# swift-nav/albatross

Hardware: AMD Instinct MI355X
Metric: GP fits/sec (Gram+Chol+solve) at N=16384 fp64 (higher is better)
Workload: dtype f64

## Files before the change

albatross_amd/csrc/chol.hip:

```cpp
#include <cstdlib>
#include "common.h"
#include "mfma_f64.h"
#include "gemm_tiles.h"
#include "trsm_kernel.h"
#include "pub.h"

namespace agp {
void launch_set_identity_batched(hipStream_t s, double *B, long long ld, long long stride, long long m, long long count);

__device__ __forceinline__ double readlane_f64(double v, int lane) {
  const long long b = __double_as_longlong(v);
  const int lo = __builtin_amdgcn_readlane((int)(b & 0xffffffffll), lane);
  const int hi = __builtin_amdgcn_readlane((int)(b >> 32), lane);
  return __longlong_as_double(((long long)hi << 32) | (unsigned int)lo);
}

__device__ __forceinline__ double rsqrt_nr(double x) {
  double y = __builtin_amdgcn_rsq(x);
  const double h = 0.5 * x;
  y = y * (1.5 - h * y * y);
  y = y * (1.5 - h * y * y);
  return y;
}

// ... 699 lines not shown
  p.A = A; p.lda = lda; p.k0 = k0; p.nbk = nbk;
  p.img = img + (k0 / NB) * (long long)IMG_DOUBLES;
  p.y = y ? y + k0 : nullptr;
  p.flags = flags; p.scalars = scalars;
  hipLaunchKernelGGL(potrf_diag_kernel, dim3(1), dim3(256), 0, s, p);
}

static void timed_gemm(hipStream_t s, FactorTimers *timers, double *C, long long lda, const double *P,
                       const double *Q, long long M, long long N, long long K, bool bulk, int variant = -1,
                       const float *P32 = nullptr, long long ld32 = 0) {
  if (!bulk) {
    launch_gemm_nt_sub(s, C, lda, P, lda, false, Q, lda, false, M, N, K, true);
    return;
  }
  BulkTiming bt;
  const bool timed = timers && timers->ev && timers->used + 2 <= timers->n_ev;
  if (timed) { bt.e0 = timers->ev[timers->used]; bt.e1 = timers->ev[timers->used + 1]; }
  if (variant >= 0) launch_trailing_update_as(variant, s, C, lda, P, Q, lda, M, K, timed ? &bt : nullptr, P32, P32, ld32);
  else launch_trailing_update(s, C, lda, P, Q, lda, M, K, timed ? &bt : nullptr);
  if (timed && bt.flops > 0.) {
    timers->flops[timers->used / 2] = bt.flops;
    timers->used += 2;
  }
}

constexpr long long FUSED_BELOW = 4608;
constexpr long long INNER_LEFT_ABOVE = 6144;
constexpr long long NBO_512_ABOVE = 2048, NBO_256_ABOVE = 1024;
constexpr long long NBO_WIDE_ABOVE = 8192;
constexpr long long THROTTLE_BELOW = 8192;
constexpr long long U1_F32_ABOVE = 4096;
constexpr long long SINGLE_BELOW = 1536;
constexpr long long MASK_BELOW = 8704;

static long long step_slots(agp_context *ctx) {
  if (ctx->step_slots <= 0) {
    int per_cu = 0;
    if (hipOccupancyMaxActiveBlocksPerMultiprocessor(&per_cu, panel_fused_kernel<true>, 256, 0) != hipSuccess || per_cu <= 0) {
      (void)hipGetLastError();
      per_cu = 1;
    }
    ctx->step_slots = (long long)per_cu * ctx->cus;
  }
  return ctx->step_slots;
}

static bool step_fits(agp_context *ctx, long long rows) {
  return ctx->tune.step_below > 0 && rows <= ctx->tune.step_below && step_slots(ctx) >= 10 + rows / 64 + 64;
}

__global__ __launch_bounds__(256) void prep_kernel(PrepArgs a) {
  int e = 0;
  while (e + 1 < a.n && (long long)blockIdx.x >= a.first_block[e + 1]) ++e;
  const long long i0 = ((long long)blockIdx.x - a.first_block[e]) * 1024 + threadIdx.x;
  unsigned long long *d = a.dst[e];
  const unsigned long long *sr = a.src[e];
  const unsigned long long pat = a.pattern[e];
#pragma unroll
  for (int u = 0; u < 4; ++u) {
    const long long i = i0 + 256 * u;
    if (i < a.count[e]) d[i] = sr ? sr[i] : pat;
  }
}

__global__ __launch_bounds__(256) void copy_table_kernel(const CopyItem *__restrict__ table) {
  const CopyItem it = table[blockIdx.y];
// ... 35 lines not shown
    ctx->d_dpub = nullptr;
    ctx->d_rowcnt = nullptr;
    ctx->dpub_cap = 0;
    const long long cap = (b1 + 31) / 32 * 32;
    if (hipMalloc(&ctx->d_dpub, sizeof(double) * (size_t)cap * (IMG_DOUBLES + 2)) == hipSuccess) {
      ctx->dpub_cap = cap;
      ctx->d_rowcnt = reinterpret_cast<unsigned long long *>(ctx->d_dpub + cap * (long long)IMG_DOUBLES);
    }
    else (void)hipGetLastError();
  }
  const long long cnt_img = (b1 - b0) * (long long)IMG_DOUBLES, cnt_z = k_end - k_begin;
  if (ctx->d_dpub && ctx->dpub_cap >= b1) {
    prep->fill(ctx->d_rowcnt + 2 * b0, 0ull, 2 * (b1 - b0));
    prep->sentinel(ctx->d_dpub + b0 * (long long)IMG_DOUBLES, cnt_img);
  }
  prep->sentinel(invd + b0 * (long long)IMG_DOUBLES, cnt_img);
  prep->sentinel(ctx->d_zpub + k_begin, cnt_z);
  if (want_step && k_begin == 0 && ctx->d_headcnt && ctx->tune.merge_above > 0 && k_end > ctx->tune.merge_above && !prep->full()) {
    prep->fill(ctx->d_headcnt, 0ull, agp_context::HEADCNT_WORDS);
    ctx->headcnt_ready = true;
  }
  ctx->zpub_ready_n = k_end;
  ctx->img_ready = invd;
  return true;
}

void panel_fused_prepare(agp_context *ctx, hipStream_t s, double *invd, long long k_begin, long long k_end, bool want_step) {
  PrepArgs prep;
  if (panel_fused_plan(ctx, invd, k_begin, k_end, want_step, &prep)) launch_prep(s, prep);
}

static void panel_phase(agp_context *ctx, hipStream_t s, double *A, long long n, long long lda, double *invd,
                        double *y, long long K0, long long kend, FactorTimers *timers, bool step_mode = false,
                        long long mark_after = -1, hipEvent_t mark_event = nullptr) {
  if (kend != n) step_mode = false;
  const bool inner_left = !step_mode && (n - K0) > INNER_LEFT_ABOVE;
  const bool fused = ctx->tune.panel_fused && ctx->d_zpub && ctx->zpub_ready_n >= kend && ctx->img_ready == invd &&
                     ((n - K0) <= FUSED_BELOW || step_mode);
  for (long long k = K0; k < kend; k += NB) {
    const int nbk = (int)((n - k < NB) ? n - k : NB);
    if (mark_event && k == mark_after + NB) (void)hipEventRecord(mark_event, s);
    if (inner_left && k > K0) {
      const double *P = A + K0 * lda + k;
      timed_gemm(s, timers, A + k * lda + k, lda, P, P, n - k, nbk, k - K0, false);
    }
    const long long below = n - (k + nbk);
    if (fused) {
      PotrfArgs pa;
      pa.A = A; pa.lda = lda; pa.k0 = k; pa.nbk = nbk;
      pa.img = invd + (k / NB) * (long long)IMG_DOUBLES;
      pa.y = y ? y + k : nullptr;
      pa.flags = ctx->d_flags; pa.scalars = ctx->d_scalars;
      pa.zpub = y ? ctx->d_zpub + k : nullptr;
      pa.below = below > 0 ? below : 0;
      if (step_mode && k > K0) {
        pa.dpub = ctx->d_dpub + (k / NB) * (long long)IMG_DOUBLES;
        unsigned grid = (unsigned)(1 + UPD_BLOCKS + (pa.below + 63) / 64);
        if (pa.below > 0) {
          const long long nt = (pa.below + 63) / 64;
          pa.trail_first = grid;
          pa.rowcnt = ctx->d_rowcnt + (k + NB) / 64;
          pa.rowcnt_expect = 2ull * (unsigned long long)((k - K0) / NB);
          const long long tiles = nt * (nt + 1) / 2 + 2 * nt;
          const long long slots = step_slots(ctx), first_round = ctx->cus, ncrit = grid;
          long long workers = tiles, nhold = 0;
          if (ncrit + workers > first_round && ncrit < first_round) {
            nhold = tiles <= 1200 ? ncrit : 1 + UPD_BLOCKS;
            const long long cap = slots - ncrit - nhold;
            if (workers > cap) workers = cap;
            if (ncrit + workers <= first_round) nhold = 0;
          } else if (workers > slots - ncrit) {
            workers = slots - ncrit;
          }
          if (workers < 2 * nt) workers = 2 * nt < tiles ? 2 * nt : tiles;
          pa.trail_tiles = tiles;
          pa.trail_workers = workers;
          grid += (unsigned)workers;
          if (nhold > 0) {
            pa.hold_index = (unsigned)first_round;
            pa.hold_count = (unsigned)nhold;
            grid += (unsigned)nhold;
          }
        }
        hipLaunchKernelGGL(panel_fused_kernel<true>, dim3(grid), dim3(256), 0, s, pa);
        ++ctx->sched.panels_step;
      } else {
        hipLaunchKernelGGL(panel_fused_kernel<false>, dim3((unsigned)(1 + (pa.below + 63) / 64)), dim3(256), 0, s, pa);
        ++ctx->sched.panels_fused;
      }
      if (below <= 0) continue;
    } else {
      launch_potrf(s, A, lda, k, nbk, invd, y, ctx->d_flags, ctx->d_scalars);
      ++ctx->sched.panels_split;
      if (below <= 0) continue;
      TrsmArgs t;
      t.img = invd + (k / NB) * (long long)IMG_DOUBLES;
      t.nbk = nbk;
      t.Y = A + k * lda + (k + nbk);
      t.stride_m = lda; t.stride_n = 1;
      t.ncols = below;
      t.z = y ? y + k : nullptr;
      t.yrest = y ? y + k + nbk : nullptr;
      t.batch_img = t.batch_Y = 0; t.n_total = 0;
      const unsigned grid = (unsigned)((below + 63) / 64);
      if (y) hipLaunchKernelGGL((trsm_micro_kernel<false, true>), dim3(grid), dim3(256), 0, s, t);
      else hipLaunchKernelGGL((trsm_micro_kernel<false, false>), dim3(grid), dim3(256), 0, s, t);
    }
    const long long width = kend - (k + nbk);
    if (width > 0 && !inner_left && !(step_mode && fused)) {
      const double *P = A + k * lda + (k + nbk);
      timed_gemm(s, timers, A + (k + nbk) * lda + (k + nbk), lda, P, P, below, width, nbk, false);
    }
  }
}

__global__ __launch_bounds__(64) void head_gate_kernel(const unsigned long long *done, unsigned long long expect, int *flags) {
  if (threadIdx.x == 0) {
    const unsigned long long t0 = __builtin_amdgcn_s_memrealtime();
    for (int spin = 1; __hip_atomic_load(done, __ATOMIC_RELAXED, __HIP_MEMORY_SCOPE_AGENT) < expect; ++spin) {
      if ((spin & 63) == 0 && poll_expired(t0, flags)) break;
      __builtin_amdgcn_s_sleep(16);
    }
    __atomic_thread_fence(__ATOMIC_ACQUIRE);
  }
}

void launch_head_gate(hipStream_t s, const unsigned long long *done, unsigned long long expect, int *flags) {
  hipLaunchKernelGGL(head_gate_kernel, dim3(1), dim3(64), 0, s, done, expect, flags);
}

static bool host_wait_event(hipEvent_t ev) {
  for (;;) {
    const hipError_t e = hipEventQuery(ev);
    if (e == hipSuccess) return true;
    if (e != hipErrorNotReady) { (void)hipGetLastError(); return false; }
    for (int i = 0; i < 32; ++i) __builtin_ia32_pause();
  }
}
// ... 127 lines not shown
      unsigned short *dst = reinterpret_cast<unsigned short *>(ctx->p32) + (size_t)(p32_flip ? 1 : 0) * (ctx->p32_bytes / sizeof(unsigned short) / 2);
      p32_flip = !p32_flip;
      launch_convert_panel_bf16x3(sa, P, lda, n - kend, K, dst);
      P16 = dst;
    } else if (variant == 5 && ctx->p32 && (n - kend) >= U1_F32_ABOVE && f16x2_depth_ok(K) && 2 * f16x2_bytes(n - kend, K) <= ctx->p32_bytes) {
      unsigned short *dst = reinterpret_cast<unsigned short *>(ctx->p32) + (size_t)(p32_flip ? 1 : 0) * (ctx->p32_bytes / sizeof(unsigned short) / 2);
      p32_flip = !p32_flip;
      launch_convert_panel_f16x2(sa, P, lda, n - kend, K, rs16 + kend, dst);
      P16 = dst;
    }
    (void)hipEventRecord(ctx->ev_a, sa);
    const bool merged = variant <= 0 && nbo_fixed == 0 && !step && next_end < n && ctx->headcnt_ready && ctx->tune.merge_above > 0 &&
                        (n - kend) > ctx->tune.merge_above && step_index < agp_context::HEADCNT_WORDS && (next_end - kend) % NB == 0;
    if (merged) {
      sb = (ctx->stream_masked && (n - kend) <= MASK_BELOW) ? ctx->stream_masked : ctx->stream2;
      if (sb != sb_prev && have_u2) (void)hipStreamWaitEvent(sb, ctx->ev_b, 0);
      sb_prev = sb;
      (void)hipStreamWaitEvent(sb, ctx->ev_a, 0);
      BulkTiming bt;
      const bool timed = timers && timers->ev && timers->used + 2 <= timers->n_ev;
      if (timed) { bt.e0 = timers->ev[timers->used]; bt.e1 = timers->ev[timers->used + 1]; }
      long long head_tiles = 0;
      unsigned long long *cnt = ctx->d_headcnt + step_index;
      launch_trailing_update_merged(sb, A + kend * lda + kend, lda, P, lda, n - kend, K, (int)((next_end - kend) / NB), cnt, &head_tiles,
                                    timed ? &bt : nullptr);
      if (timed && bt.flops > 0.) {
        timers->flops[timers->used / 2] = bt.flops;
        timers->used += 2;
      }
      (void)hipEventRecord(ctx->ev_b, sb);
      have_u2 = true;
      launch_head_gate(sa, cnt, (unsigned long long)head_tiles, ctx->d_flags);
      rec.add_step(next_end, rec.MERGED | (sb == ctx->stream_masked ? rec.MASKED : 0u));
      panel_phase(ctx, sa, A, n, lda, invd, y, kend, next_end, timers, false);
      K0 = kend;
      kend = next_end;
      ++step_index;
      continue;
    }
    ++step_index;
    if (have_u2) (void)hipStreamWaitEvent(sa, ctx->ev_b, 0);
    if (P16 && variant == 5) {
      launch_update_f16x2(sa, A + kend * lda + kend, lda, P16, n - kend, 0, 0, irs16 + kend, n - kend, next_end - kend, K);
    } else if (P16) {
      launch_update_bf16x3(sa, A + kend * lda + kend, lda, P16, n - kend, 0, 0, n - kend, next_end - kend, K);
    } else if ((variant == 3 || variant == 4 || variant == 5) && (n - kend) >= U1_F32_ABOVE) {
      launch_update_f32(sa, A + kend * lda + kend, lda, P, P, lda, n - kend, next_end - kend, K, P32, P32, ld32);
    } else if (step && n - kend > 1536) {
      timed_gemm(sa, timers, A + kend * lda + kend, lda, P, P, n - kend, n - kend, K, true, variant >= 4 ? 3 : variant);
    } else {
      timed_gemm(sa, timers, A + kend * lda + kend, lda, P, P, n - kend, next_end - kend, K, false);
    }
    sb = (ctx->stream_masked && (n - kend) <= MASK_BELOW) ? ctx->stream_masked : ctx->stream2;
    if (sb != sb_prev && have_u2) (void)hipStreamWaitEvent(sb, ctx->ev_b, 0);
    sb_prev = sb;
    const bool throttle = next_end < n && (n - kend) <= THROTTLE_BELOW;
    rec.add_step(next_end, (step ? rec.STEP : 0u) | (throttle ? rec.THROTTLED : 0u) | (single ? rec.SINGLE : 0u) |
                               (next_end < n && sb == ctx->stream_masked ? rec.MASKED : 0u));
    if (throttle) panel_phase(ctx, sa, A, n, lda, invd, y, kend, next_end, timers, step);
    if (next_end < n) {
      if (throttle) {
        if (!host_wait_event(ctx->ev_a)) (void)hipStreamWaitEvent(sb, ctx->ev_a, 0);
      } else {
        (void)hipStreamWaitEvent(sb, ctx->ev_a, 0);
      }
      const double *Q = A + K0 * lda + next_end;
      if (P16) {
// ... 162 lines not shown
```

albatross_amd/csrc/common.h:

```cpp
#pragma once
#include <hip/hip_runtime.h>
#include <cstdint>
#include <cstdio>
#include <string>
#include <utility>
#include <vector>

#include "../../include/albatross_amd.h"
#include "cov_eval.h"

#define AGP_CHAIN_PRIO 3

namespace agp {

constexpr int NB = 128;
constexpr int NBO = 512;
constexpr int MB = 16;
constexpr int NMB = NB / MB;

struct FeatView {
  const double *coords;
  const long long *ids;
  const double *scales;
  long long n;
// ... 74 lines not shown
  struct Tuning {
    bool panel_fused = true;
    long long step_below = 4608;
    bool gram_sop = true;
    long long fp64_nbo = 0;
    long long mixed_nbo = 512;
    bool mixed_f16 = true;
    bool mixed_bf16 = true;
    long long backsub_coop_max = 2047;
    bool backsub_coop = true;
    bool sparse_pivoted = false;
    long long predict_chunk = 0;
    long long shard_block = 0;
    bool shard_force_comm = false;
    bool shard_host_pacing = false;
    double shard_mask_gflop = 40.;
    long long merge_above = 8704;
  } tune;
  unsigned long long *d_rowcnt = nullptr;
  void *h_stage = nullptr;
  size_t h_stage_bytes = 0;
  static constexpr long long HEADCNT_WORDS = 256;
  unsigned long long *d_headcnt = nullptr;
  bool headcnt_ready = false;
  struct ScheduleRecord {
    static constexpr unsigned MERGED = 1, STEP = 2, THROTTLED = 4, MASKED = 8, SINGLE = 16;
    enum Backsub { BS_NONE = 0, BS_COOP_DIRECT = 1, BS_COOP_FLAGS = 2, BS_WIDE = 3, BS_CHAIN = 4 };
    static constexpr unsigned INV_EARLY = 1, INV_LAST_STEP = 2, INV_TAIL = 4;
    long long n = 0;
    long long steps = 0, steps_dropped = 0;
    long long kend[HEADCNT_WORDS] = {};
    unsigned bits[HEADCNT_WORDS] = {};
    long long panels_step = 0, panels_fused = 0, panels_split = 0;
    int backsub = BS_NONE;
    long long bs_done = 0;
    unsigned inv_bits = 0;
    int handover_timeout = 0;
    long long demotions = 0;
    void reset_factor(long long n_) {
      n = n_;
      steps = steps_dropped = 0;
      panels_step = panels_fused = panels_split = 0;
      inv_bits = 0;
      handover_timeout = 0;
    }
    void add_step(long long end, unsigned b) {
      if (steps < HEADCNT_WORDS) { kend[steps] = end; bits[steps] = b; ++steps; }
      else ++steps_dropped;
    }
  } sched;
  double *bs_W = nullptr;
  long long bs_BW = 0, bs_done = 0;
  hipEvent_t ev_inv = nullptr;
  const double *img_ready = nullptr;
  bool prep_external = false;
  hipStream_t stream_comm = nullptr;
  unsigned long long *shard_flags = nullptr;
  unsigned long long shard_seq[16] = {};
  unsigned long long shard_probe_seq = 0;
  int shard_host_pacing = -1;
  bool shard_probe_ok = false;
};

struct agp_fit_slab {
  double *base = nullptr;
  size_t bytes = 0;
  int refs = 0;
};

struct agp_fit {
  agp_context *ctx = nullptr;
  agp_fit_slab *slab = nullptr;
  size_t A_bytes = 0;
  int device = 0;
  int64_t n = 0;
// ... 79 lines not shown
void right_solve_lt_batched(hipStream_t s, const double *A, long long stride_A, long long n, long long lda,
                            const double *invd, long long stride_invd, double *X, long long stride_X, long long nrows,
                            long long ldx, long long count);
void launch_gemm_nt_sub_batched(hipStream_t s, double *C, long long ldc, long long batch_C, const double *A,
                                long long lda, bool a_kmajor, long long batch_A, const double *B, long long ldb,
                                bool b_kmajor, long long batch_B, long long M, long long N, long long K, bool tri,
                                long long count);
void right_solve_lt(hipStream_t s, const double *A, long long n, long long lda, const double *invd, double *X,
                    long long nrows, long long ldx);
void forward_solve_mat_lookahead(agp_context *ctx, const double *A, long long n, long long lda, const double *invd,
                                 double *B, long long m, long long ldb, bool rhs_lower = false);
void backward_solve_mat(hipStream_t s, const double *A, long long n, long long lda, const double *invd,
                        double *B, long long m, long long ldb);
constexpr long long WIDE_BW = 512;
bool forward_solve_wide_ok(long long n, long long ncols);
void invert_wide_blocks(hipStream_t s, const double *A, long long n, long long lda, const double *invd, long long BW, double *W);
void forward_solve_wide(hipStream_t s, const double *A, long long n, long long lda, const double *Winv, const double *B,
                        long long ldb, double *X, long long ldx, long long ncols);

void launch_coldot(hipStream_t s, const double *A, long long lda, const double *B, long long ldb,
                   long long n, long long m, double *out, double scale, const double *base);
void launch_gemm_tn_sub(hipStream_t s, const double *V, long long ldv, const double *W, long long ldw,
                        long long n, long long m, double *C, long long ldc);
void launch_gemv_t(hipStream_t s, const double *A, long long lda, long long n, long long m,
                   const double *x, double *y);
void launch_dot(hipStream_t s, const double *a, const double *b, long long n, double *out);

}

namespace agp {
void launch_gemm_nt_sub(hipStream_t s, double *C, long long ldc, const double *A, long long lda,
                        bool a_kmajor, const double *B, long long ldb, bool b_kmajor, long long M,
                        long long N, long long K, bool tri);
void launch_gemm_nt_ext(hipStream_t s, double *C, long long ldc, const double *Cin, long long ldcin, const double *A, long long lda,
                        const double *B, long long ldb, long long M, long long N, long long K);
void launch_gemm_nt_sub_stair(hipStream_t s, double *C, long long ldc, const double *A, long long lda, const double *B,
                              long long ldb, long long M, long long N, long long K, int world, int rank, long long lb0,
                              long long block, long long c0);
struct BulkTiming {
  hipEvent_t e0 = nullptr, e1 = nullptr;
  double flops = 0.;
};
void launch_trailing_update_as(int variant, hipStream_t s, double *C, long long ldc, const double *P,
                               const double *Q, long long ldp, long long M, long long K,
                               BulkTiming *timing = nullptr, const float *P32 = nullptr, const float *Q32 = nullptr,
                               long long ld32 = 0);
void launch_trailing_update(hipStream_t s, double *C, long long ldc, const double *P, const double *Q,
                            long long ldp, long long M, long long K, BulkTiming *timing = nullptr);
void read_bulk_probe(unsigned long long *out);
void read_bf16_probe(unsigned long long *out);
void read_potrf_probe(unsigned long long *out);
void launch_head_gate(hipStream_t s, const unsigned long long *done, unsigned long long expect, int *flags);
void launch_trailing_update_merged(hipStream_t s, double *C, long long ldc, const double *P, long long ldp, long long M, long long K,
                                   int head_cols, unsigned long long *head_done, long long *head_tiles, BulkTiming *timing = nullptr);
void launch_update_f32(hipStream_t s, double *C, long long ldc, const double *P, const double *Q, long long ldp, long long M,
                       long long N, long long K, const float *P32 = nullptr, const float *Q32 = nullptr, long long ld32 = 0);
size_t bf16x3_bytes(long long rows, long long K);
void launch_convert_panel_bf16x3(hipStream_t s, const double *P, long long ldp, long long rows, long long K, unsigned short *planes);
void set_bf16x3_kernel(int choice, int lds_pad);
void launch_update_bf16x3(hipStream_t s, double *C, long long ldc, const unsigned short *planes, long long panel_rows, long long row_a,
                          long long row_b, long long M, long long N, long long K, const int *order = nullptr, long long order_len = 0);
size_t f16x2_bytes(long long rows, long long K);
void launch_f16x2_row_scales(hipStream_t s, const double *A, long long lda, long long n, double *rs, double *irs);
void launch_convert_panel_f16x2(hipStream_t s, const double *P, long long ldp, long long rows, long long K, const double *rs,
                                unsigned short *planes);
void set_f16x2_kernel(int lds_pad, int terms, int chunk);
// ... 8 lines not shown
```

albatross_amd/csrc/debug_api.hip:

```cpp
#include <algorithm>
#include <cstdio>
#include "common.h"
#include "api_internal.h"
#include "mfma_f64.h"
#include "shard_internal.h"
#include <cstdlib>
#include <cstring>
#include <new>

#define AGP_DEBUG_API __attribute__((visibility("default")))

namespace agp {

__global__ void mfma_tile_kernel(const double *A, const double *B, double *D) {
  const int l = threadIdx.x;
  v4d acc = v4zero();
  acc = mfma16(A[(l & 15) * 4 + (l >> 4)], B[(l >> 4) * 16 + (l & 15)], acc);
  for (int r = 0; r < 4; ++r) D[((l >> 4) + 4 * r) * 16 + (l & 15)] = acc[r];
}

template <int NACC>
__global__ __launch_bounds__(256) void mfma_clock_kernel(unsigned long long *out, int iters, double a0, double b0) {
  v4d acc[NACC];
#pragma unroll
  for (int i = 0; i < NACC; ++i) acc[i] = v4zero();
  const double a = a0 * (1.0 + (threadIdx.x % 7) * 0.125), b = b0 * (1.0 - (threadIdx.x % 5) * 0.0625);
  const unsigned long long c0 = __builtin_amdgcn_s_memtime();
  const unsigned long long r0 = __builtin_amdgcn_s_memrealtime();
  for (int it = 0; it < iters; ++it) {
#pragma unroll
    for (int i = 0; i < NACC; ++i) acc[i] = mfma16(a, b, acc[i]);
  }
  double s = 0.;
#pragma unroll
  for (int i = 0; i < NACC; ++i) s += acc[i][0] + acc[i][3];
  const unsigned long long c1 = __builtin_amdgcn_s_memtime();
  const unsigned long long r1 = __builtin_amdgcn_s_memrealtime();
  if (threadIdx.x == 0) {
// ... 450 lines not shown
  for (int i = 0; i < nblk; ++i) {
    cyc[i] = (double)h[2 * i] / (double)iters;
    clk[i] = (double)h[2 * i] / ((double)h[2 * i + 1] * 10.0);
  }
  std::sort(cyc.begin(), cyc.end());
  std::sort(clk.begin(), clk.end());
  out[0] = cyc[nblk / 2];
  out[1] = clk[nblk / 2];
  out[2] = (double)nblk * 4.0 * iters * (nm * 2048.0 + nv * 128.0) / (ms * 1e-3) / 1e12;
  out[3] = nm; out[4] = nv;
  (void)hipEventDestroy(e0); (void)hipEventDestroy(e1); (void)hipFree(d);
  return AGP_OK;
}

AGP_DEBUG_API int agp_debug_gemm(agp_context *ctx, double *C, int64_t ldc, const double *A, int64_t lda, int a_kmajor,
                   const double *B, int64_t ldb, int b_kmajor, int64_t M, int64_t N, int64_t K, int tri) {
  if (!ctx) return AGP_ERR_INVALID_ARGUMENT;
  AGP_HIP_CHECK(ctx, hipSetDevice(ctx->device));
  const size_t cb = sizeof(double) * (size_t)ldc * (size_t)N;
  const size_t ab = sizeof(double) * (size_t)lda * (size_t)(a_kmajor ? M : K);
  const size_t bb = sizeof(double) * (size_t)ldb * (size_t)(b_kmajor ? N : K);
  double *dC = nullptr, *dA = nullptr, *dB = nullptr;
  AGP_HIP_CHECK(ctx, hipMalloc(&dC, cb));
  AGP_HIP_CHECK(ctx, hipMalloc(&dA, ab));
  AGP_HIP_CHECK(ctx, hipMalloc(&dB, bb));
  AGP_HIP_CHECK(ctx, hipMemcpy(dC, C, cb, hipMemcpyHostToDevice));
  AGP_HIP_CHECK(ctx, hipMemcpy(dA, A, ab, hipMemcpyHostToDevice));
  AGP_HIP_CHECK(ctx, hipMemcpy(dB, B, bb, hipMemcpyHostToDevice));
  launch_gemm_nt_sub(ctx->stream, dC, ldc, dA, lda, a_kmajor != 0, dB, ldb, b_kmajor != 0, M, N, K, tri != 0);
  AGP_HIP_CHECK(ctx, hipStreamSynchronize(ctx->stream));
  AGP_HIP_CHECK(ctx, hipGetLastError());
  AGP_HIP_CHECK(ctx, hipMemcpy(C, dC, cb, hipMemcpyDeviceToHost));
  (void)hipFree(dC); (void)hipFree(dA); (void)hipFree(dB);
  return AGP_OK;
}

AGP_DEBUG_API int agp_debug_fmac_rate(agp_context *ctx, int waves_per_simd, int mode, int iters, double *out, double *probe) {
  if (!ctx) return AGP_ERR_INVALID_ARGUMENT;
  AGP_HIP_CHECK(ctx, hipSetDevice(ctx->device));
  const int nblk = 256 * waves_per_simd;
  unsigned long long *d = nullptr;
  double *dp = nullptr;
  AGP_HIP_CHECK(ctx, hipMalloc(&d, sizeof(unsigned long long) * 2 * nblk));
  AGP_HIP_CHECK(ctx, hipMalloc(&dp, sizeof(double) * 64));
  hipEvent_t e0, e1;
  AGP_HIP_CHECK(ctx, hipEventCreate(&e0));
  AGP_HIP_CHECK(ctx, hipEventCreate(&e1));
  for (int rep = 0; rep < 2; ++rep) {
    AGP_HIP_CHECK(ctx, hipEventRecord(e0, ctx->stream));
    if (mode == 0) hipLaunchKernelGGL(fmac_rate_kernel<0>, dim3(nblk), dim3(256), 0, ctx->stream, d, dp, iters, 1.1);
    else if (mode == 1) hipLaunchKernelGGL(fmac_rate_kernel<1>, dim3(nblk), dim3(256), 0, ctx->stream, d, dp, iters, 1.1);
    else hipLaunchKernelGGL(fmac_rate_kernel<2>, dim3(nblk), dim3(256), 0, ctx->stream, d, dp, iters, 1.1);
    AGP_HIP_CHECK(ctx, hipEventRecord(e1, ctx->stream));
    AGP_HIP_CHECK(ctx, hipEventSynchronize(e1));
  }
  float ms = 0.f;
  AGP_HIP_CHECK(ctx, hipEventElapsedTime(&ms, e0, e1));
  std::vector<unsigned long long> h(2 * nblk);
  AGP_HIP_CHECK(ctx, hipMemcpy(h.data(), d, sizeof(unsigned long long) * 2 * nblk, hipMemcpyDeviceToHost));
  if (probe) AGP_HIP_CHECK(ctx, hipMemcpy(probe, dp, sizeof(double) * 64, hipMemcpyDeviceToHost));
  std::vector<double> cyc(nblk), clk(nblk);
  for (int i = 0; i < nblk; ++i) {
    cyc[i] = (double)h[2 * i] / (double)iters;
    clk[i] = (double)h[2 * i] / ((double)h[2 * i + 1] * 10.0);
  }
  std::sort(cyc.begin(), cyc.end());
// ... 302 lines not shown
    AGP_HIP_CHECK(ctx, hipMemcpy(dy, y, sizeof(double) * (size_t)n, hipMemcpyHostToDevice));
  }
  AGP_HIP_CHECK(ctx, hipMemsetAsync(ctx->d_flags, 0, 4 * sizeof(int), ctx->stream));
  AGP_HIP_CHECK(ctx, hipMemsetAsync(ctx->d_scalars, 0, 4 * sizeof(double), ctx->stream));
  factor_lower(ctx, dA, n, lda, dI, dy, nullptr);
  AGP_HIP_CHECK(ctx, hipStreamSynchronize(ctx->stream));
  AGP_HIP_CHECK(ctx, hipGetLastError());
  AGP_HIP_CHECK(ctx, hipMemcpy(A, dA, ab, hipMemcpyDeviceToHost));
  if (y) AGP_HIP_CHECK(ctx, hipMemcpy(y, dy, sizeof(double) * (size_t)n, hipMemcpyDeviceToHost));
  int flags[4];
  double scal[4];
  AGP_HIP_CHECK(ctx, hipMemcpy(flags, ctx->d_flags, sizeof(flags), hipMemcpyDeviceToHost));
  AGP_HIP_CHECK(ctx, hipMemcpy(scal, ctx->d_scalars, sizeof(scal), hipMemcpyDeviceToHost));
  if (log_det) *log_det = 2. * scal[0];
  if (bad_pivot) *bad_pivot = flags[1] ? flags[1] - 1 : -1;
  (void)hipFree(dA); (void)hipFree(dI);
  if (dy) (void)hipFree(dy);
  ctx->sched.backsub = agp_context::ScheduleRecord::BS_NONE;
  ctx->sched.bs_done = 0;
  ctx->sched.handover_timeout = flags[2];
  return AGP_OK;
}

constexpr int64_t SCHED_HEADER = 20;
AGP_DEBUG_API int agp_debug_schedule(agp_context *ctx, int64_t *out, int64_t cap) {
  if (!ctx || !out || cap < 0) return AGP_ERR_INVALID_ARGUMENT;
  const agp_context::ScheduleRecord &r = ctx->sched;
  int64_t w[SCHED_HEADER + 2 * agp_context::HEADCNT_WORDS] = {};
  w[0] = r.n; w[1] = r.steps; w[2] = r.steps_dropped;
  w[3] = r.panels_step; w[4] = r.panels_fused; w[5] = r.panels_split;
  w[6] = r.backsub; w[7] = r.bs_done; w[8] = r.inv_bits; w[9] = r.handover_timeout; w[10] = r.demotions;
  w[11] = ctx->step_slots; w[12] = ctx->cus; w[13] = ctx->stream_masked ? 1 : 0;
  w[14] = ctx->tune.step_below; w[15] = ctx->tune.panel_fused ? 1 : 0; w[16] = ctx->tune.merge_above;
  w[17] = ctx->tune.backsub_coop ? 1 : 0; w[18] = ctx->tune.fp64_nbo;
  for (long long i = 0; i < r.steps; ++i) {
    w[SCHED_HEADER + 2 * i] = r.kend[i];
    w[SCHED_HEADER + 2 * i + 1] = r.bits[i];
  }
  const int64_t total = SCHED_HEADER + 2 * agp_context::HEADCNT_WORDS;
  for (int64_t i = 0; i < cap && i < total; ++i) out[i] = w[i];
  return AGP_OK;
}

}

namespace agp {
__global__ __launch_bounds__(256) void mfma_peak_kernel(double *sink, int iters, double a0, double b0) {
  v4d acc[8];
#pragma unroll
  for (int i = 0; i < 8; ++i) acc[i] = v4zero();
  double a = a0 + threadIdx.x * 1e-9, b = b0 - threadIdx.x * 1e-9;
  for (int it = 0; it < iters; ++it) {
#pragma unroll
    for (int i = 0; i < 8; ++i) acc[i] = mfma16(a, b, acc[i]);
  }
  double s = 0.;
#pragma unroll
  for (int i = 0; i < 8; ++i) s += acc[i][0] + acc[i][1] + acc[i][2] + acc[i][3];
  if (s == 123.456) sink[0] = s;
}

static int mfma_f64_peak(hipStream_t s, int iters, double *tflops) {
  double *sink = nullptr;
  if (hipMalloc(&sink, 8) != hipSuccess) return AGP_ERR_HIP;
  hipEvent_t e0, e1;
  (void)hipEventCreate(&e0);
  (void)hipEventCreate(&e1);
// ... 70 lines not shown
```

albatross_amd/csrc/gemm.hip:

```cpp
#include <cmath>
#include <cstdlib>
#include <algorithm>
#include <map>
#include <mutex>
#include <tuple>
#include <vector>
#include "common.h"
#include "mfma_f64.h"
#include "gemm_tiles.h"

namespace agp {




__device__ __forceinline__ bool tile_of_block(const GemmArgs &g, int &bi, int &bj) {
  if (g.stair) {
    const long long id = blockIdx.x;
    bi = (int)(id % g.ntr);
    bj = (int)(id / g.ntr);
    const long long lb = g.st_lb0 + bi / g.st_tpb;
    const long long gi = lb * g.st_world + ((lb & 1) ? g.st_world - 1 - g.st_rank : g.st_rank);
    return bj <= gi * g.st_tpb - g.st_c0t + (bi % g.st_tpb);
  }
// ... 456 lines not shown
  g.ntc = (int)((N + GT - 1) / GT);
  g.stair = 1; g.st_world = world; g.st_rank = rank; g.st_tpb = (int)(block / GT);
  g.st_lb0 = lb0; g.st_c0t = c0 / GT;
  static int slots = 0;
  if (slots == 0) {
    int dev = 0, cus = 256;
    if (hipGetDevice(&dev) != hipSuccess || hipDeviceGetAttribute(&cus, hipDeviceAttributeMultiprocessorCount, dev) != hipSuccess || cus <= 0)
      cus = 256;
    slots = 2 * cus;
  }
  if ((long long)g.ntr * g.ntc / 2 < 4LL * slots) {
    g.ntr = (int)((M + ST - 1) / ST);
    g.ntc = (int)((N + ST - 1) / ST);
    g.st_tpb = (int)(block / ST);
    g.st_c0t = c0 / ST;
    hipLaunchKernelGGL(gemm64_nt_sub_kernel, dim3((unsigned)((long long)g.ntr * g.ntc)), dim3(GEMM_THREADS), 0, s, g);
    return;
  }
  hipLaunchKernelGGL((gemm_nt_sub_kernel<false, false>), dim3((unsigned)((long long)g.ntr * g.ntc)), dim3(GEMM_THREADS), 0, s, g);
}

void launch_gemm_nt_ext(hipStream_t s, double *C, long long ldc, const double *Cin, long long ldcin, const double *A, long long lda,
                        const double *B, long long ldb, long long M, long long N, long long K) {
  if (M <= 0 || N <= 0 || K <= 0) return;
  GemmArgs g;
  g.C = C; g.ldc = ldc; g.A = A; g.lda = lda; g.B = B; g.ldb = ldb;
  g.M = M; g.N = N; g.K = K; g.tri = 0;
  g.ntr = (int)((M + GT - 1) / GT);
  g.ntc = (int)((N + GT - 1) / GT);
  g.Cin = Cin; g.ldcin = ldcin; g.assign = Cin ? 0 : 1;
  hipLaunchKernelGGL(gemm_nt_ext_kernel, dim3((unsigned)((long long)g.ntr * g.ntc)), dim3(GEMM_THREADS), 0, s, g);
}

void launch_gemm_nt_sub(hipStream_t s, double *C, long long ldc, const double *A, long long lda,
                        bool a_kmajor, const double *B, long long ldb, bool b_kmajor, long long M,
                        long long N, long long K, bool tri) {
  launch_gemm_nt_sub_batched(s, C, ldc, 0, A, lda, a_kmajor, 0, B, ldb, b_kmajor, 0, M, N, K, tri, 1);
}

static double lower_entries(long long M, int ntr, long long count) {
  double e = 0.;
  for (int bj = 0; bj < ntr && count > 0; ++bj) {
    const long long w = (M - (long long)bj * GT < GT) ? M - (long long)bj * GT : GT;
    for (int bi = bj; bi < ntr && count > 0; ++bi, --count) {
      const long long h = (M - (long long)bi * GT < GT) ? M - (long long)bi * GT : GT;
      e += (bi == bj) ? 0.5 * (double)w * (double)(w + 1) : (double)h * (double)w;
    }
  }
  return e;
}

struct XcdOrder { int *dev = nullptr; long long len = 0; };
static XcdOrder xcd_order(int ntr, long long full) {
  static std::mutex mu;
  static std::map<std::tuple<int, int, long long>, XcdOrder> cache;
  int device = 0;
  (void)hipGetDevice(&device);
  std::lock_guard<std::mutex> lock(mu);
  auto key = std::make_tuple(device, ntr, full);
  auto it = cache.find(key);
  if (it != cache.end()) return it->second;
  constexpr int SB = 8, XCDS = 8;
  auto index_of = [&](int bi, int bj) { return (long long)bj * ntr - (long long)bj * (bj - 1) / 2 + (bi - bj); };
  const int nsb = (ntr + SB - 1) / SB;
  std::vector<std::vector<int>> blocks;
  for (int SJ = 0; SJ < nsb; ++SJ)
// ... 174 lines not shown
```

albatross_amd/csrc/trsm_kernel.h:

```cpp
#pragma once
#include "common.h"
#include "mfma_f64.h"

namespace agp {

constexpr int NTILE = NMB * (NMB + 1) / 2;
constexpr int IMG_DOUBLES = NTILE * MB * MB;

__device__ __forceinline__ int tile_off(int ib, int kb) { return (ib * (ib + 1) / 2 + kb) * (MB * MB); }

constexpr int NFRAG_TILES = NTILE;

struct TrsmArgs {
  const double *img;
  int nbk;
  double *Y;
  long long stride_m, stride_n;
  long long ncols;
  const double *z;
  double *yrest;
  long long batch_img, batch_Y;
  long long n_total;
  long long batch_z = 0;
};
// ... 63 lines not shown
#pragma unroll
      for (int ib = NMB - 1; ib > jb; --ib) {
        const double *f = F + (ib * (ib + 1) / 2 + jb) * 256 + lane;
#pragma unroll
        for (int s = 0; s < 4; ++s) pa[s] = mfma16(f[s * 64], Y[ib][s], pa[s]);
      }
      const v4d acc = (pa[0] + pa[1]) + (pa[2] + pa[3]);
      v4d po[4] = {v4zero(), v4zero(), v4zero(), v4zero()};
      const double *f = F + (jb * (jb + 1) / 2 + jb) * 256 + lane;
#pragma unroll
      for (int s = 0; s < 4; ++s) po[s] = mfma16(f[s * 64], acc[s], po[s]);
      const v4d out = (po[0] + po[1]) + (po[2] + po[3]);
      Y[jb] = out;
#pragma unroll
      for (int r = 0; r < 4; ++r) {
        const int m = jb * MB + lg + 4 * r;
        if (nok && m < p.nbk) base[m * p.stride_m] = out[r];
      }
    }
  }

  if (FUSE_Y) {
    double part = 0.;
#pragma unroll
    for (int jb = 0; jb < NMB; ++jb)
#pragma unroll
      for (int r = 0; r < 4; ++r) part += Y[jb][r] * zs[jb * MB + lg + 4 * r];
    part += __shfl_xor(part, 16, 64);
    part += __shfl_xor(part, 32, 64);
    if (lg == 0 && nok) p.yrest[n0 + ln] -= part;
  }
}


template <int CTRL>
__device__ __forceinline__ double dpp_move(double v) {
  int lo = __double2loint(v), hi = __double2hiint(v);
  lo = __builtin_amdgcn_mov_dpp(lo, CTRL, 0xF, 0xF, true);
  hi = __builtin_amdgcn_mov_dpp(hi, CTRL, 0xF, 0xF, true);
  return __hiloint2double(hi, lo);
}
template <int MASK>
__device__ __forceinline__ double row_xor(double v) {
  static_assert(MASK == 1 || MASK == 2 || MASK == 4 || MASK == 8, "inside a row of 16 lanes");
  if (MASK == 1) return dpp_move<0xB1>(v);
  if (MASK == 2) return dpp_move<0x4E>(v);
  if (MASK == 4) return dpp_move<0x1B>(dpp_move<0x141>(v));
  return dpp_move<0x141>(dpp_move<0x140>(v));
}

template <class Emit>
__device__ __forceinline__ void micro_backsub_wave(const double *F, const double *ts, Emit emit) {
  const int lane = threadIdx.x & 63;
  const int k = lane >> 2, mq = lane & 3;
  double t[NMB];
#pragma unroll
  for (int jb = 0; jb < NMB; ++jb) t[jb] = ts[jb * MB + k];
#pragma unroll
  for (int jb = NMB - 1; jb >= 0; --jb) {
    const double *D = F + tile_off(jb, jb) + k * MB + 4 * mq;
    double part = 0.;
#pragma unroll
    for (int u = 0; u < 4; ++u) part += D[u] * __shfl(t[jb], (4 * mq + u) << 2, 64);
    part += row_xor<1>(part);
    part += row_xor<2>(part);
    const double xk = part;
// ... 32 lines not shown
#undef AGP_COLSUM_STEP
  double sum = acc[0];
  sum += __shfl_xor(sum, 16, 64);
  sum += __shfl_xor(sum, 32, 64);
  return sum;
}
__device__ __forceinline__ int colsum16_index(int lane) {
  return ((lane & 1) << 3) | ((lane & 2) << 1) | ((lane & 4) >> 1) | ((lane & 8) >> 3);
}

template <bool TRANS, bool FUSE_Y>
__global__ __launch_bounds__(256, 2) void trsm_micro_kernel(TrsmArgs p) {
  __builtin_amdgcn_s_setprio(AGP_CHAIN_PRIO);
  __shared__ double F[NFRAG_TILES * 4 * 64 + NB];
  double *zs = F + NFRAG_TILES * 4 * 64;
  if (blockIdx.y > 0 || p.n_total > 0) {
    const long long b = blockIdx.y;
    p.img += b * p.batch_img;
    p.Y += b * p.batch_Y;
    if (FUSE_Y) {
      p.z += b * p.batch_z;
      p.yrest += b * p.batch_z;
    }
    if (p.n_total > 0) {
      const long long left = p.n_total - b * NB;
      p.nbk = (int)(left < NB ? left : NB);
    }
  }
  trsm_micro_stage<TRANS, FUSE_Y>(p, F, zs);
  __syncthreads();
  trsm_micro_solve<TRANS, FUSE_Y>(p, F, zs, ((long long)blockIdx.x * 4 + (threadIdx.x >> 6)) * 16);
}

}
```

Before: 34.63.

## Add lean chain path with dense persistent TRSM and direct 128-tile GEMM

For early merged steps with a large remaining trailing matrix, the panel phase now calls a direct 128-tile NT GEMM launcher for the inner left-looking update, bypassing timed_gemm's dispatch and timing. It also replaces the per-64-row TRSM grid with a fixed-size persistent kernel, where each wave solves two 16-column groups at once with MFMA. The aim is to cut launch overhead and let the panel-chain kernels take fewer CUs while the concurrent trailing update runs. In exchange the TRSM has less parallelism per launch, and timers no longer record these GEMMs.

```diff
diff --git a/albatross_amd/csrc/chol.hip b/albatross_amd/csrc/chol.hip
--- a/albatross_amd/csrc/chol.hip
+++ b/albatross_amd/csrc/chol.hip
@@ -755,6 +755,13 @@
 constexpr long long U1_F32_ABOVE = 4096;
 constexpr long long SINGLE_BELOW = 1536;
 constexpr long long MASK_BELOW = 8704;
+#ifndef AGP_DENSE_CHAIN_ABOVE
+#define AGP_DENSE_CHAIN_ABOVE 11264
+#endif
+constexpr long long DENSE_CHAIN_ABOVE = AGP_DENSE_CHAIN_ABOVE;
+#ifndef AGP_LEAN_INNER
+#define AGP_LEAN_INNER 1
+#endif
 
 static long long step_slots(agp_context *ctx) {
   if (ctx->step_slots <= 0) {
@@ -856,9 +863,10 @@
 
 static void panel_phase(agp_context *ctx, hipStream_t s, double *A, long long n, long long lda, double *invd,
                         double *y, long long K0, long long kend, FactorTimers *timers, bool step_mode = false,
-                        long long mark_after = -1, hipEvent_t mark_event = nullptr) {
+                        long long mark_after = -1, hipEvent_t mark_event = nullptr, bool lean = false) {
   if (kend != n) step_mode = false;
   const bool inner_left = !step_mode && (n - K0) > INNER_LEFT_ABOVE;
+  lean = lean && inner_left;
   const bool fused = ctx->tune.panel_fused && ctx->d_zpub && ctx->zpub_ready_n >= kend && ctx->img_ready == invd &&
                      ((n - K0) <= FUSED_BELOW || step_mode);
   for (long long k = K0; k < kend; k += NB) {
@@ -866,7 +874,8 @@
     if (mark_event && k == mark_after + NB) (void)hipEventRecord(mark_event, s);
     if (inner_left && k > K0) {
       const double *P = A + K0 * lda + k;
-      timed_gemm(s, timers, A + k * lda + k, lda, P, P, n - k, nbk, k - K0, false);
+      if (lean && AGP_LEAN_INNER) launch_gemm_nt_sub_128(s, A + k * lda + k, lda, P, lda, P, lda, n - k, nbk, k - K0, true);
+      else timed_gemm(s, timers, A + k * lda + k, lda, P, P, n - k, nbk, k - K0, false);
     }
     const long long below = n - (k + nbk);
     if (fused) {
@@ -927,7 +936,11 @@
       t.yrest = y ? y + k + nbk : nullptr;
       t.batch_img = t.batch_Y = 0; t.n_total = 0;
       const unsigned grid = (unsigned)((below + 63) / 64);
-      if (y) hipLaunchKernelGGL((trsm_micro_kernel<false, true>), dim3(grid), dim3(256), 0, s, t);
+      if (lean && grid > (unsigned)TRSM_DENSE_WGS && nbk == NB && below + NB * lda <= 0xffffffffLL) {
+        ++ctx->sched.panels_dense;
+        if (y) hipLaunchKernelGGL((trsm_rows_dense_kernel<true>), dim3(TRSM_DENSE_WGS), dim3(256), 0, s, t);
+        else hipLaunchKernelGGL((trsm_rows_dense_kernel<false>), dim3(TRSM_DENSE_WGS), dim3(256), 0, s, t);
+      } else if (y) hipLaunchKernelGGL((trsm_micro_kernel<false, true>), dim3(grid), dim3(256), 0, s, t);
       else hipLaunchKernelGGL((trsm_micro_kernel<false, false>), dim3(grid), dim3(256), 0, s, t);
     }
     const long long width = kend - (k + nbk);
@@ -1121,7 +1134,7 @@
       have_u2 = true;
       launch_head_gate(sa, cnt, (unsigned long long)head_tiles, ctx->d_flags);
       rec.add_step(next_end, rec.MERGED | (sb == ctx->stream_masked ? rec.MASKED : 0u));
-      panel_phase(ctx, sa, A, n, lda, invd, y, kend, next_end, timers, false);
+      panel_phase(ctx, sa, A, n, lda, invd, y, kend, next_end, timers, false, -1, nullptr, (n - kend) > DENSE_CHAIN_ABOVE);
       K0 = kend;
       kend = next_end;
       ++step_index;
diff --git a/albatross_amd/csrc/common.h b/albatross_amd/csrc/common.h
--- a/albatross_amd/csrc/common.h
+++ b/albatross_amd/csrc/common.h
@@ -130,6 +130,7 @@
     long long kend[HEADCNT_WORDS] = {};
     unsigned bits[HEADCNT_WORDS] = {};
     long long panels_step = 0, panels_fused = 0, panels_split = 0;
+    long long panels_dense = 0;
     int backsub = BS_NONE;
     long long bs_done = 0;
     unsigned inv_bits = 0;
@@ -138,7 +139,7 @@
     void reset_factor(long long n_) {
       n = n_;
       steps = steps_dropped = 0;
-      panels_step = panels_fused = panels_split = 0;
+      panels_step = panels_fused = panels_split = panels_dense = 0;
       inv_bits = 0;
       handover_timeout = 0;
     }
@@ -284,6 +285,8 @@
 void launch_gemm_nt_sub(hipStream_t s, double *C, long long ldc, const double *A, long long lda,
                         bool a_kmajor, const double *B, long long ldb, bool b_kmajor, long long M,
                         long long N, long long K, bool tri);
+void launch_gemm_nt_sub_128(hipStream_t s, double *C, long long ldc, const double *A, long long lda, const double *B,
+                            long long ldb, long long M, long long N, long long K, bool tri);
 void launch_gemm_nt_ext(hipStream_t s, double *C, long long ldc, const double *Cin, long long ldcin, const double *A, long long lda,
                         const double *B, long long ldb, long long M, long long N, long long K);
 void launch_gemm_nt_sub_stair(hipStream_t s, double *C, long long ldc, const double *A, long long lda, const double *B,
diff --git a/albatross_amd/csrc/debug_api.hip b/albatross_amd/csrc/debug_api.hip
--- a/albatross_amd/csrc/debug_api.hip
+++ b/albatross_amd/csrc/debug_api.hip
@@ -4,6 +4,7 @@
 #include "api_internal.h"
 #include "mfma_f64.h"
 #include "shard_internal.h"
+#include "trsm_kernel.h"
 #include <cstdlib>
 #include <cstring>
 #include <new>
@@ -520,6 +521,68 @@
   AGP_HIP_CHECK(ctx, hipGetLastError());
   AGP_HIP_CHECK(ctx, hipMemcpy(C, dC, cb, hipMemcpyDeviceToHost));
   (void)hipFree(dC); (void)hipFree(dA); (void)hipFree(dB);
+  return AGP_OK;
+}
+
+AGP_DEBUG_API int agp_debug_gemm128(agp_context *ctx, double *C, int64_t ldc, const double *A, int64_t lda, const double *B,
+                                    int64_t ldb, int64_t M, int64_t N, int64_t K, int tri) {
+  if (!ctx || M <= 0 || N <= 0 || K <= 0 || ldc < M || lda < M || ldb < N) return AGP_ERR_INVALID_ARGUMENT;
+  AGP_HIP_CHECK(ctx, hipSetDevice(ctx->device));
+  const size_t cb = sizeof(double) * (size_t)ldc * (size_t)N, ab = sizeof(double) * (size_t)lda * (size_t)K,
+               bb = sizeof(double) * (size_t)ldb * (size_t)K;
+  double *dC = nullptr, *dA = nullptr, *dB = nullptr;
+  AGP_HIP_CHECK(ctx, hipMalloc(&dC, cb));
+  AGP_HIP_CHECK(ctx, hipMalloc(&dA, ab));
+  AGP_HIP_CHECK(ctx, hipMalloc(&dB, bb));
+  AGP_HIP_CHECK(ctx, hipMemcpy(dC, C, cb, hipMemcpyHostToDevice));
+  AGP_HIP_CHECK(ctx, hipMemcpy(dA, A, ab, hipMemcpyHostToDevice));
+  AGP_HIP_CHECK(ctx, hipMemcpy(dB, B, bb, hipMemcpyHostToDevice));
+  launch_gemm_nt_sub_128(ctx->stream, dC, ldc, dA, lda, dB, ldb, M, N, K, tri != 0);
+  AGP_HIP_CHECK(ctx, hipStreamSynchronize(ctx->stream));
+  AGP_HIP_CHECK(ctx, hipGetLastError());
+  AGP_HIP_CHECK(ctx, hipMemcpy(C, dC, cb, hipMemcpyDeviceToHost));
+  (void)hipFree(dC); (void)hipFree(dA); (void)hipFree(dB);
+  return AGP_OK;
+}
+
+AGP_DEBUG_API int agp_debug_panel_trsm(agp_context *ctx, const double *img, double *X, int64_t ld, int64_t rows, const double *z,
+                                       double *yrest, int dense, int wgs) {
+  if (!ctx || !img || !X || rows <= 0 || ld < rows || (z && !yrest) || rows + (int64_t)NB * ld > 0xffffffffLL) return AGP_ERR_INVALID_ARGUMENT;
+  AGP_HIP_CHECK(ctx, hipSetDevice(ctx->device));
+  const size_t xb = sizeof(double) * (size_t)ld * NB, ib = sizeof(double) * (size_t)IMG_DOUBLES;
+  double *dX = nullptr, *dI = nullptr, *dz = nullptr, *dy = nullptr;
+  AGP_HIP_CHECK(ctx, hipMalloc(&dX, xb));
+  AGP_HIP_CHECK(ctx, hipMalloc(&dI, ib));
+  AGP_HIP_CHECK(ctx, hipMemcpy(dX, X, xb, hipMemcpyHostToDevice));
+  AGP_HIP_CHECK(ctx, hipMemcpy(dI, img, ib, hipMemcpyHostToDevice));
+  if (z) {
+    AGP_HIP_CHECK(ctx, hipMalloc(&dz, sizeof(double) * NB));
+    AGP_HIP_CHECK(ctx, hipMalloc(&dy, sizeof(double) * (size_t)rows));
+    AGP_HIP_CHECK(ctx, hipMemcpy(dz, z, sizeof(double) * NB, hipMemcpyHostToDevice));
+    AGP_HIP_CHECK(ctx, hipMemcpy(dy, yrest, sizeof(double) * (size_t)rows, hipMemcpyHostToDevice));
+  }
+  TrsmArgs t;
+  t.img = dI; t.nbk = NB;
+  t.Y = dX; t.stride_m = ld; t.stride_n = 1;
+  t.ncols = rows;
+  t.z = dz; t.yrest = dy;
+  t.batch_img = t.batch_Y = 0; t.n_total = 0;
+  hipStream_t s = ctx->stream;
+  if (dense) {
+    const unsigned g = (unsigned)(wgs > 0 ? wgs : TRSM_DENSE_WGS);
+    if (z) hipLaunchKernelGGL((trsm_rows_dense_kernel<true>), dim3(g), dim3(256), 0, s, t);
+    else hipLaunchKernelGGL((trsm_rows_dense_kernel<false>), dim3(g), dim3(256), 0, s, t);
+  } else {
+    const unsigned g = (unsigned)((rows + 63) / 64);
+    if (z) hipLaunchKernelGGL((trsm_micro_kernel<false, true>), dim3(g), dim3(256), 0, s, t);
+    else hipLaunchKernelGGL((trsm_micro_kernel<false, false>), dim3(g), dim3(256), 0, s, t);
+  }
+  AGP_HIP_CHECK(ctx, hipStreamSynchronize(s));
+  AGP_HIP_CHECK(ctx, hipGetLastError());
+  AGP_HIP_CHECK(ctx, hipMemcpy(X, dX, xb, hipMemcpyDeviceToHost));
+  if (z) AGP_HIP_CHECK(ctx, hipMemcpy(yrest, dy, sizeof(double) * (size_t)rows, hipMemcpyDeviceToHost));
+  (void)hipFree(dX); (void)hipFree(dI);
+  if (z) { (void)hipFree(dz); (void)hipFree(dy); }
   return AGP_OK;
 }
 
@@ -888,7 +951,7 @@
   w[6] = r.backsub; w[7] = r.bs_done; w[8] = r.inv_bits; w[9] = r.handover_timeout; w[10] = r.demotions;
   w[11] = ctx->step_slots; w[12] = ctx->cus; w[13] = ctx->stream_masked ? 1 : 0;
   w[14] = ctx->tune.step_below; w[15] = ctx->tune.panel_fused ? 1 : 0; w[16] = ctx->tune.merge_above;
-  w[17] = ctx->tune.backsub_coop ? 1 : 0; w[18] = ctx->tune.fp64_nbo;
+  w[17] = ctx->tune.backsub_coop ? 1 : 0; w[18] = ctx->tune.fp64_nbo; w[19] = r.panels_dense;
   for (long long i = 0; i < r.steps; ++i) {
     w[SCHED_HEADER + 2 * i] = r.kend[i];
     w[SCHED_HEADER + 2 * i + 1] = r.bits[i];
diff --git a/albatross_amd/csrc/gemm.hip b/albatross_amd/csrc/gemm.hip
--- a/albatross_amd/csrc/gemm.hip
+++ b/albatross_amd/csrc/gemm.hip
@@ -512,6 +512,20 @@
   hipLaunchKernelGGL(gemm_nt_ext_kernel, dim3((unsigned)((long long)g.ntr * g.ntc)), dim3(GEMM_THREADS), 0, s, g);
 }
 
+void launch_gemm_nt_sub_128(hipStream_t s, double *C, long long ldc, const double *A, long long lda, const double *B,
+                            long long ldb, long long M, long long N, long long K, bool tri) {
+  if (M <= 0 || N <= 0 || K <= 0) return;
+  GemmArgs g;
+  g.C = C; g.ldc = ldc; g.A = A; g.lda = lda; g.B = B; g.ldb = ldb;
+  g.M = M; g.N = N; g.K = K; g.tri = tri ? 1 : 0;
+  g.ntr = (int)((M + GT - 1) / GT);
+  g.ntc = (int)((N + GT - 1) / GT);
+  if (tri && g.ntc > g.ntr) g.ntc = g.ntr;
+  const long long tiles = count_tiles(g.ntr, g.ntc, g.tri);
+  if (tiles <= 0) return;
+  hipLaunchKernelGGL((gemm_nt_sub_kernel<false, false>), dim3((unsigned)tiles), dim3(GEMM_THREADS), 0, s, g);
+}
+
 void launch_gemm_nt_sub(hipStream_t s, double *C, long long ldc, const double *A, long long lda,
                         bool a_kmajor, const double *B, long long ldb, bool b_kmajor, long long M,
                         long long N, long long K, bool tri) {
diff --git a/albatross_amd/csrc/trsm_kernel.h b/albatross_amd/csrc/trsm_kernel.h
--- a/albatross_amd/csrc/trsm_kernel.h
+++ b/albatross_amd/csrc/trsm_kernel.h
@@ -119,6 +119,83 @@
   }
 }
 
+template <bool FUSE_Y, int NG>
+__device__ __forceinline__ void trsm_micro_solve_multi(const TrsmArgs &p, const double *F, const double *zs, const long long (&n0)[NG]) {
+  const int lane = threadIdx.x & 63;
+  const int ln = lane & 15, lg = lane >> 4;
+  unsigned sm = (unsigned)p.stride_m;
+  __asm__ volatile("" : "+s"(sm));
+  bool nok[NG];
+  unsigned col[NG];
+  v4d Y[NG][NMB];
+#pragma unroll
+  for (int g = 0; g < NG; ++g) {
+    nok[g] = n0[g] + ln < p.ncols;
+    col[g] = nok[g] ? (unsigned)(n0[g] + ln) : 0u;
+  }
+#pragma unroll
+  for (int g = 0; g < NG; ++g)
+#pragma unroll
+    for (int jb = 0; jb < NMB; ++jb)
+#pragma unroll
+      for (int r = 0; r < 4; ++r) {
+        const int m = jb * MB + lg + 4 * r;
+        Y[g][jb][r] = nok[g] ? p.Y[col[g] + (unsigned)m * sm] : 0.;
+      }
+#pragma unroll
+  for (int jb = 0; jb < NMB; ++jb) {
+    v4d pa[NG][4];
+#pragma unroll
+    for (int g = 0; g < NG; ++g) {
+      pa[g][0] = Y[g][jb];
+      pa[g][1] = pa[g][2] = pa[g][3] = v4zero();
+    }
+#pragma unroll
+    for (int ib = 0; ib < jb; ++ib) {
+      const double *f = F + (jb * (jb + 1) / 2 + ib) * 256 + lane;
+#pragma unroll
+      for (int s = 0; s < 4; ++s)
+#pragma unroll
+        for (int g = 0; g < NG; ++g) pa[g][s] = mfma16(f[s * 64], Y[g][ib][s], pa[g][s]);
+    }
+    v4d acc[NG], po[NG][4];
+#pragma unroll
+    for (int g = 0; g < NG; ++g) {
+      acc[g] = (pa[g][0] + pa[g][1]) + (pa[g][2] + pa[g][3]);
+      po[g][0] = po[g][1] = po[g][2] = po[g][3] = v4zero();
+    }
+    const double *f = F + (jb * (jb + 1) / 2 + jb) * 256 + lane;
+#pragma unroll
+    for (int s = 0; s < 4; ++s)
+#pragma unroll
+      for (int g = 0; g < NG; ++g) po[g][s] = mfma16(f[s * 64], acc[g][s], po[g][s]);
+#pragma unroll
+    for (int g = 0; g < NG; ++g) {
+      const v4d out = (po[g][0] + po[g][1]) + (po[g][2] + po[g][3]);
+      Y[g][jb] = out;
+#pragma unroll
+      for (int r = 0; r < 4; ++r) {
+        const int m = jb * MB + lg + 4 * r;
+        if (nok[g]) p.Y[col[g] + (unsigned)m * sm] = out[r];
+      }
+    }
+  }
+
+  if (FUSE_Y) {
+#pragma unroll
+    for (int g = 0; g < NG; ++g) {
+      double part = 0.;
+#pragma unroll
+      for (int jb = 0; jb < NMB; ++jb)
+#pragma unroll
+        for (int r = 0; r < 4; ++r) part += Y[g][jb][r] * zs[jb * MB + lg + 4 * r];
+      part += __shfl_xor(part, 16, 64);
+      part += __shfl_xor(part, 32, 64);
+      if (lg == 0 && nok[g]) p.yrest[n0[g] + ln] -= part;
+    }
+  }
+}
+
 
 template <int CTRL>
 __device__ __forceinline__ double dpp_move(double v) {
@@ -217,4 +294,26 @@
   trsm_micro_solve<TRANS, FUSE_Y>(p, F, zs, ((long long)blockIdx.x * 4 + (threadIdx.x >> 6)) * 16);
 }
 
-}
+constexpr int TRSM_DENSE_NG = 2;
+#ifndef AGP_TRSM_DENSE_WGS
+#define AGP_TRSM_DENSE_WGS 64
+#endif
+constexpr int TRSM_DENSE_WGS = AGP_TRSM_DENSE_WGS;
+
+template <bool FUSE_Y>
+__global__ __launch_bounds__(256, 2) void trsm_rows_dense_kernel(TrsmArgs p) {
+  __builtin_amdgcn_s_setprio(AGP_CHAIN_PRIO);
+  __shared__ double F[NFRAG_TILES * 4 * 64 + NB];
+  double *zs = F + NFRAG_TILES * 4 * 64;
+  trsm_micro_stage<false, FUSE_Y>(p, F, zs);
+  __syncthreads();
+  const long long waves = (long long)gridDim.x * 4, groups = (p.ncols + 15) / 16;
+  for (long long g = (long long)blockIdx.x * 4 + (threadIdx.x >> 6); g < groups; g += TRSM_DENSE_NG * waves) {
+    long long n0[TRSM_DENSE_NG];
+#pragma unroll
+    for (int i = 0; i < TRSM_DENSE_NG; ++i) n0[i] = (g + i * waves) * 16;
+    trsm_micro_solve_multi<FUSE_Y, TRSM_DENSE_NG>(p, F, zs, n0);
+  }
+}
+
+}
```

After: 34.90, median of 6. No clear change (+0.8%).
